# y9c/cutseq

Hardware: AMD Instinct MI355X
Metric: M read-pairs/sec (higher is better)
Workload: dtype u8

## Files before the change

### cutseq_amd/capi.py

```python
from __future__ import annotations

import ctypes as C
from pathlib import Path

from . import abi, switches

LIB_PATH = Path(__file__).with_name("libcutseq_hip.so")

EXPORTS = (
    "cs_abi_version", "cs_last_error", "cs_device_count", "cs_plan_create", "cs_plan_destroy", "cs_plan_set_demux", "cs_plan_set_demux_ops", "cs_plan_set_max_n",
    "cs_plan_set_max_length", "cs_plan_set_max_ee", "cs_plan_set_ee_reversed", "cs_xflag_counts_fetch", "cs_text_discards",
    "cs_engine_create", "cs_engine_destroy", "cs_trim_device", "cs_trim_device_pipelined", "cs_join", "cs_trim_batch", "cs_sync",
    "cs_stats_fetch", "cs_last_kernel_ms", "cs_last_kernel_split_ms", "cs_kernel_time_totals", "cs_alloc_pinned", "cs_alloc_pinned_huge", "cs_free_pinned", "cs_alloc_device",
    "cs_free_device", "cs_copy_to_device", "cs_copy_to_host",
    "cs_text_create", "cs_text_destroy", "cs_text_submit", "cs_text_wait", "cs_text_routes", "cs_text_fetch",
    "cs_text_info", "cs_text_fetch_info",
)


class HipUnavailable(RuntimeError):
    """The HIP extension (or a usable MI355X) is missing; the product has no CPU path."""


class CsError(RuntimeError):
    def __init__(self, code: int, message: str):
        super().__init__(f"cutseq_hip error {code}: {message}")
        self.code = code


_lib = None


def load() -> C.CDLL:
    global _lib
    if _lib is not None:
        return _lib
    lib_path = Path(switches.path("HIP_LIB", str(LIB_PATH)))
    if not lib_path.exists():
        raise HipUnavailable(
            f"{lib_path} not found: build it with `python -m cutseq_amd.build` "
            "(hipcc --offload-arch=gfx950). cutseq_amd has no CPU trimming path."
        )
    try:
        L = C.CDLL(str(lib_path))
    except OSError as exc:
        raise HipUnavailable(f"cannot load {lib_path}: {exc}") from exc
    vp, u32, i32 = C.c_void_p, C.c_uint32, C.c_int
    L.cs_abi_version.restype = i32
    L.cs_last_error.restype = C.c_char_p
    L.cs_device_count.restype = i32
    L.cs_plan_create.restype = i32
    L.cs_plan_create.argtypes = [vp, i32, vp, i32, C.POINTER(abi.cs_params), C.POINTER(vp)]
    L.cs_plan_set_demux.restype = i32
    L.cs_plan_set_demux.argtypes = [vp, i32, i32, vp, C.c_size_t]
    L.cs_plan_set_demux_ops.restype = i32
    L.cs_plan_set_demux_ops.argtypes = [vp, i32, i32, vp, i32]
    L.cs_plan_set_max_n.restype = i32
    L.cs_plan_set_max_n.argtypes = [vp, C.c_double]
    L.cs_plan_set_max_length.restype = i32
    L.cs_plan_set_max_length.argtypes = [vp, C.c_uint32]
    L.cs_plan_set_max_ee.restype = i32
    L.cs_plan_set_max_ee.argtypes = [vp, C.c_double]
    L.cs_plan_set_ee_reversed.restype = i32
    L.cs_plan_set_ee_reversed.argtypes = [vp, i32]
    L.cs_xflag_counts_fetch.restype = i32
    L.cs_xflag_counts_fetch.argtypes = [vp, vp, i32]
    L.cs_text_discards.restype = i32
    L.cs_text_discards.argtypes = [vp, C.c_uint32, vp]
    L.cs_plan_destroy.restype = None
    L.cs_plan_destroy.argtypes = [vp]
    L.cs_engine_create.restype = i32
    L.cs_engine_create.argtypes = [vp, i32, u32, u32, u32, C.POINTER(vp)]
    L.cs_engine_destroy.restype = None
    L.cs_engine_destroy.argtypes = [vp]
    L.cs_trim_device.restype = i32
    L.cs_trim_device.argtypes = [vp, vp, C.POINTER(abi.cs_reads), C.POINTER(abi.cs_reads), u32, u32]
    L.cs_trim_device_pipelined.restype = i32
    L.cs_trim_device_pipelined.argtypes = [vp, vp, C.POINTER(abi.cs_reads), C.POINTER(abi.cs_reads), u32, u32]
    L.cs_join.restype = i32
    L.cs_join.argtypes = [vp, vp]
    L.cs_trim_batch.restype = i32
    L.cs_trim_batch.argtypes = [vp, u32, C.POINTER(abi.cs_reads), C.POINTER(abi.cs_reads), u32, u32]
    L.cs_sync.restype = i32
    L.cs_sync.argtypes = [vp, u32]
    L.cs_stats_fetch.restype = i32
    L.cs_stats_fetch.argtypes = [vp, C.POINTER(abi.cs_stats * 2), i32]
    L.cs_last_kernel_ms.restype = i32
    L.cs_last_kernel_ms.argtypes = [vp, C.POINTER(C.c_float)]
    L.cs_last_kernel_split_ms.restype = i32
    L.cs_last_kernel_split_ms.argtypes = [vp, C.POINTER(C.c_float * 2)]
    L.cs_kernel_time_totals.restype = i32
    L.cs_kernel_time_totals.argtypes = [vp, C.POINTER(u32), C.POINTER(C.c_float * 2), i32]
    L.cs_alloc_pinned.restype = vp
    L.cs_alloc_pinned.argtypes = [C.c_size_t]
    L.cs_alloc_pinned_huge.restype = vp
    L.cs_alloc_pinned_huge.argtypes = [C.c_size_t]
    L.cs_free_pinned.restype = None
    L.cs_free_pinned.argtypes = [vp]
    L.cs_alloc_device.restype = vp
    L.cs_alloc_device.argtypes = [i32, C.c_size_t]
    L.cs_free_device.restype = None
    L.cs_free_device.argtypes = [i32, vp]
    L.cs_copy_to_device.restype = i32
    L.cs_copy_to_device.argtypes = [i32, vp, vp, C.c_size_t]
    L.cs_copy_to_host.restype = i32
    L.cs_copy_to_host.argtypes = [i32, vp, vp, C.c_size_t]
    u64 = C.c_uint64
    L.cs_text_create.restype = i32
    L.cs_text_create.argtypes = [vp, C.POINTER(abi.cs_text_params), u32, u64, u32, u32, C.POINTER(vp)]
    L.cs_text_destroy.restype = None
    L.cs_text_destroy.argtypes = [vp]
    L.cs_text_submit.restype = i32
    L.cs_text_submit.argtypes = [vp, u32, vp, u64, vp, u64, u32]
    L.cs_text_wait.restype = i32
    L.cs_text_wait.argtypes = [vp, u32, C.POINTER(abi.cs_text_result)]
    L.cs_text_routes.restype = i32
    L.cs_text_routes.argtypes = [vp, u32, vp, vp, vp]
# ... 27 lines not shown
```

### cutseq_amd/csrc/cutseq_hip.hip

```cpp
#include <hip/hip_runtime.h>

#include <cmath>
#include <cstdarg>
#include <cstdio>
#include <cstdlib>
#include <cstring>
#include <algorithm>
#include <atomic>
#include <map>
#include <new>
#include <string>
#include <thread>
#include <vector>

#include <sys/mman.h>

#include "../../include/cutseq_hip.h"
#include "trim_kernel.hip.inc"
#include "long_kernel.hip.inc"
#include "text_kernels.hip.inc"
#include "deflate_kernels.hip.inc"
#include "info_kernels.hip.inc"

namespace {
// ... 491 lines not shown
          d.fnib[idx >> 3] |= (uint32_t)((d.op.seq[d.op.reversed ? mm - 1 - idx : idx] >> 3) & 7u) << (4 * (idx & 7));
    }
  for (int m = 0; m < 2; ++m)
    for (int i = 0; i < cnt[m]; ++i) {
      csdev::DevOp &d = p->host.ops[m][i];
      if (d.op.kind != CS_OP_CUT) continue;
      auto pack = [](const cs_op &o) {
        return (uint32_t)(uint16_t)o.cut_len | ((uint32_t)(o.conditional ? 1u : 0u) << 16) | ((uint32_t)(o.capture & 3u) << 17) |
               ((uint32_t)(o.force_min_len > 0x1fff ? 0x1fffu : o.force_min_len) << 19);
      };
      d.cut_run = 1;
      d.cut_pack[0] = pack(d.op);
    }
  {
    const char *env = getenv("CUTSEQ_CUT_RUNS");
    if (!(env && atoi(env) == 0))
      for (int m = 0; m < 2; ++m)
        for (int i = 0; i < cnt[m];) {
          if (p->host.ops[m][i].op.kind != CS_OP_CUT) {
            ++i;
            continue;
          }
          int j = i;
          while (j < cnt[m] && j - i < csdev::kCutRun && p->host.ops[m][j].op.kind == CS_OP_CUT) {
            p->host.ops[m][i].cut_pack[j - i] = p->host.ops[m][j].cut_pack[0];
            ++j;
          }
          p->host.ops[m][i].cut_run = (uint32_t)(j - i);
          i = j;
        }
  }
  {
    const char *env = getenv("CUTSEQ_PAIR");
    const bool allow = coded && !(env && atoi(env) == 0);
    const char *env_log = getenv("CUTSEQ_LOG_ALWAYS");
    const bool log_always = env_log && atoi(env_log) != 0;
    auto log_friendly = [log_always](int mm, int kk) {
      if (log_always) return true;
      double variants = 0, choose = 1, pw = 1;
      for (int e = 0; e <= kk && e <= mm; ++e) {
        variants += choose * pw;
        choose = choose * (double)(mm - e) / (double)(e + 1);
        pw *= 6.0;
      }
      double space = 1;
      for (int i = 0; i < mm; ++i) space *= 4.0;
      return 300.0 * variants / space < 0.03;
    };
    for (int m = 0; m < 2; ++m) {
      if (allow && cnt[m] >= 1) {
        csdev::DevOp &f = p->host.ops[m][0];
        const bool free_ends = (f.op.align_flags & (CS_QUERY_START | CS_QUERY_STOP)) == (CS_QUERY_START | CS_QUERY_STOP);
        if (f.op.kind == CS_OP_ADAPTER && f.filter_mode == csdev::FILTER_MYERS32 && !f.op.reversed && free_ends &&
            f.op.shortcut == CS_SHORTCUT_NONE && !f.exists_only && log_friendly(f.op.m, f.op.k))
          f.solo_first = 1;
      }
      if (!allow || cnt[m] < 2) continue;
      csdev::DevOp &a = p->host.ops[m][0];
      const csdev::DevOp &b = p->host.ops[m][1];
      const int ma = a.op.m, ka = a.op.k, mo = a.op.min_overlap;
      const bool ends_free = (b.op.align_flags & (CS_QUERY_START | CS_QUERY_STOP)) == (CS_QUERY_START | CS_QUERY_STOP);
      if (!a.exists_only || a.op.kind != CS_OP_ADAPTER || b.op.kind != CS_OP_ADAPTER || b.exists_only ||
          b.filter_mode != csdev::FILTER_MYERS32 || b.op.reversed || !ends_free || b.op.shortcut != CS_SHORTCUT_NONE ||
          ma + ka > 31 || ka > 14 || !log_friendly(b.op.m, b.op.k))
        continue;
      a.pair_next = 1;
      for (int ent = 0; ent < 4; ++ent) {
        const int which = (ent == 0) ? 0 : (ent == 1) ? 1 : (ent == 2) ? 3 : 2;
        uint32_t fwd = 0;
        for (int i = 0; i < ma; ++i)
          if ((a.peq[which] >> (ma - 1 - i)) & 1ull) fwd |= 1u << i;
        a.eq_fwd[ent] = fwd << (32 - ma);
      }
      for (int j = 1; j <= 32; ++j) {
        int best = -1;
        if (j > ma + ka) best = ka;
        else
          for (int i = mo; i <= ma; ++i) {
            const int d = i > j ? i - j : j - i;
            if (d <= (int)a.op.thr[i] && (int)a.op.thr[i] > best) best = a.op.thr[i];
          }
        a.pair_tn[(j - 1) >> 3] |= (uint32_t)(best + 1) << (4 * ((j - 1) & 7));
      }
    }
  }
  *out = p;
  return CS_OK;
}

void cs_plan_destroy(cs_plan *plan) { delete plan; }

int cs_plan_set_max_n(cs_plan *plan, double count) {
  if (!plan) return fail(CS_ERR_ARG, "null plan");
  if (!(count >= 0.0)) return fail(CS_ERR_ARG, "max_n %g: the count must not be negative or NaN", count);
  plan->host.max_n_on = 1;
  plan->host.max_n = count;
  return CS_OK;
}

int cs_plan_set_max_length(cs_plan *plan, uint32_t length) {
  if (!plan) return fail(CS_ERR_ARG, "null plan");
  plan->host.max_length_on = 1;
  plan->host.max_length = length;
  return CS_OK;
}

int cs_plan_set_max_ee(cs_plan *plan, double errors) {
  if (!plan) return fail(CS_ERR_ARG, "null plan");
  if (!(errors >= 0.0)) return fail(CS_ERR_ARG, "max_ee %g: the bound must not be negative or NaN", errors);
  plan->host.max_ee_on = 1;
  plan->host.max_ee = errors;
  for (int b = 0; b < 256; ++b) plan->host.ee_table[b] = pow(10.0, (double)(33 - b) / 10.0);
  return CS_OK;
}

int cs_plan_set_ee_reversed(cs_plan *plan, int reversed) {
  if (!plan) return fail(CS_ERR_ARG, "null plan");
  plan->host.ee_reversed = reversed ? 1u : 0u;
  return CS_OK;
}

int cs_plan_set_demux(cs_plan *plan, int mate, int op_index, const uint16_t *table, size_t entries) {
  if (!plan || !table) return fail(CS_ERR_ARG, "null plan or table");
  if (mate < 1 || mate > 2 || op_index < 0 || op_index >= plan->host.n_ops[mate - 1])
    return fail(CS_ERR_ARG, "mate %d op %d: no such op", mate, op_index);
  const cs_op &op = plan->host.ops[mate - 1][op_index].op;
  if (op.kind != CS_OP_DEMUX) return fail(CS_ERR_ARG, "mate %d op %d is not a CS_OP_DEMUX op", mate, op_index);
  if (plan->host.ops[mate - 1][op_index].filter_mode)
    return fail(CS_ERR_ARG, "mate %d op %d: m + k = %d > %d (or CS_DEMUX_BY_OPS) takes cs_plan_set_demux_ops, not a table", mate,
                op_index, op.m + op.k, CS_DEMUX_MAX_PREFIX);
  size_t want = 0, pw = 1;
  for (int l = 0; l <= op.m + op.k; ++l, pw *= 5) want += pw;
  if (entries != want) return fail(CS_ERR_ARG, "demux table: %zu entries, expected %zu for m + k = %d", entries, want, op.m + op.k);
  try {
    plan->demux[mate - 1][op_index].assign(table, table + entries);
  } catch (const std::bad_alloc &) {
    return fail(CS_ERR_NOMEM, "out of memory");
  }
  return CS_OK;
}

namespace {

struct DemuxSegment {
  std::vector<uint8_t> pool;
  std::vector<std::pair<size_t, uint32_t>> first;
};

struct DemuxWalk {
  const std::vector<std::string> &digits;
  int m, k, depth;
  const std::vector<size_t> &block;

  struct Alive {
    int id;
    bool done;
    uint8_t col[CS_MAX_ADAPTER + 1];
  };
  struct Task {
    int len;
    size_t idx, pw, segment;
    std::vector<Alive> alive;
  };
  std::vector<std::vector<Alive>> scratch;
  DemuxSegment *seg = nullptr;
  bool overflow = false;
  int split = -1;
  std::vector<DemuxSegment> *segments = nullptr;
  std::vector<Task> *tasks = nullptr;

  void emit(size_t at, const std::vector<Alive> &alive) {
// ... 1299 lines not shown
```

### cutseq_amd/csrc/trim_kernel.hip.inc

```

#include <type_traits>

namespace csdev {

#ifdef CS_PHASE_TIMERS
struct PhaseTimer {
  uint64_t last;
  uint32_t acc[8];
  uint32_t passes, steps, items;
};
#define CS_T_MARK(T, PHASE)                                   \
  {                                                           \
    const uint64_t cs_now = clock64();                        \
    (T).acc[PHASE] += (uint32_t)(cs_now - (T).last);          \
    (T).last = cs_now;                                        \
  }
#else
#define CS_T_MARK(T, PHASE)
#endif


constexpr int kWave = 64;

constexpr uint32_t kScoreBias = 1024u, kOriginBias = 4096u;
constexpr uint32_t kCostShift = 24, kScoreShift = 13;
constexpr uint32_t kCellZero = (kScoreBias << kScoreShift) | kOriginBias;
constexpr uint32_t kDeltaMatch = 1u << kScoreShift;
constexpr uint32_t kDeltaMismatch = (1u << kCostShift) - (1u << kScoreShift);
constexpr uint32_t kDeltaIndel = (1u << kCostShift) - (2u << kScoreShift);

enum { FILTER_NONE = 0, FILTER_MYERS32 = 1, FILTER_MYERS64 = 2, FILTER_POLY_TAIL = 3, FILTER_POLY_HEAD = 4 };

__host__ __device__ constexpr uint32_t base_code(uint32_t ascii) {
  const uint32_t sel = (ascii >> 1) & 3u;
  const bool ok = ascii == 'A' || ascii == 'C' || ascii == 'G' || ascii == 'T';
  return (sel << 3) | (ok ? 0u : 32u);
}
constexpr int kEqTableBytes = 64;
constexpr int kWaveItemDwords = 4;
constexpr int kCutRun = 4;
constexpr int kQCutoffLow = -1, kQCutoffHigh = 256, kQTermMax = 256;

struct DevFields {
  uint32_t kind, align_flags, reversed, remove, shortcut, match_flag, required, conditional, capture, homopolymer,
      q_base, stat_slot, m, k, min_overlap, force_min_len;
  int32_t cut_len, q_cutoff;
};

struct DevOp {
  cs_op op;
  DevFields f;
  uint64_t peq[4];
  uint32_t filter_mode;
  uint32_t base_char;
  uint32_t acgt_only;
  uint32_t thr_mul;
  uint64_t thr_step[2];
  uint32_t eq_tab[kEqTableBytes / 4];
  uint32_t fnib[6];
  uint32_t exists_only;
  uint32_t pair_next;
  uint32_t solo_first;
  uint32_t pair_tn[4];
  uint32_t eq_fwd[4];
  uint32_t cut_run;
  uint32_t cut_pack[kCutRun];
};

struct DevPlan {
  cs_params params;
  int32_t n_ops[2];
  int32_t coded;
  int32_t max_n_on;
  DevOp ops[2][CS_MAX_OPS];
  double max_n;
  uint32_t max_length_on, max_length;
  uint32_t max_ee_on, ee_reversed;
  double max_ee;
  double ee_table[256];
};

constexpr int kMaxPlanSlots = 8;
__constant__ DevPlan c_plans[kMaxPlanSlots];

struct MateArgs {
  const uint32_t *seq;
  const uint8_t *qual;
  const uint16_t *len;
  cs_result *out;
  cs_cap2 *cap2;
  uint8_t *bc;
  uint8_t *xflags;
};

constexpr uint32_t kTileCounters = 8, kTileCounterStride = 32;

struct KArgs {
  MateArgs mate[2];
  unsigned long long *stats;
  uint32_t n_reads;
  uint32_t stride_dw;
  uint32_t lds_stride_dw;
  uint32_t col_dwords;
  uint32_t plan_slot;
  uint32_t *tile_counter;
  uint32_t n_table_ops;
  uint32_t big_tiles;
  uint32_t big_shift, small_shift;
  uint32_t static_units;
  uint4 *defer[2];
  uint32_t batch_knob;
  uint32_t *defer_count;
  uint32_t defer_cap;
  const unsigned long long *gate;
  uint32_t item_slots;
  uint32_t fast_recode;
};

__device__ __forceinline__ uint32_t cell_pack(int cost, int score, int origin) {
  return ((uint32_t)cost << kCostShift) | ((uint32_t)(score + (int)kScoreBias) << kScoreShift) |
// ... 881 lines not shown
  const uint32_t fill_a = (uint32_t)sha, cst4 = (uint32_t)(4 + 2 * ka + 1);
  auto sample_a = [&](uint32_t cst) {
    const int cur = (int)__builtin_popcount(sa.Pv) - (int)(__builtin_popcount(sa.Mv) + fill_a);
    flag |= sa.score + cur - (int)cst;
    sa.score = cur;
  };
  const unsigned long long tn_lo = ((unsigned long long)tn1 << 32) | tn0, tn_hi = ((unsigned long long)tn3 << 32) | tn2;
  auto tn_of = [tn_lo, tn_hi, ka](int j) -> int {
    int t1 = ka + 1;
    if (__ballot(j <= 32)) {
      const unsigned long long w = j <= 16 ? tn_lo : tn_hi;
      const int tj = (int)((uint32_t)(w >> (((uint32_t)(j - 1) & 15u) * 4u)) & 15u);
      t1 = j > 32 ? t1 : tj;
    }
    return t1;
  };
  auto column = [&](uint32_t eb, uint32_t ea, int j) {
    myers_step_la<false>(st, eb, 0u);
    if constexpr (HAS_A) {
      myers_step_la<false>(sa, ea, 0u);
      flag |= sa.score - tn_of(j);
    }
    if (st.score < 0) {
      if (jfirst < 0) jfirst = j;
      jlast = j;
      if (j == jmin + 1 && st.score + k1 == cmin) tie_next = true;
      if (st.score + k1 < cmin) {
        cmin = st.score + k1;
        jmin = j;
        tie_next = false;
      }
    }
  };
  int j = 1;
  if (n >= NB) {
    int wi = 0;
    auto take = [&]() -> uint32_t { return row[wi]; };
    auto advance = [&]() { wi += 1; };
#ifndef CS_PAIR_DEPTH
#define CS_PAIR_DEPTH 2
#endif
    constexpr int QD = CS_PAIR_DEPTH;
    static_assert(NB % QD == 0, "a group's columns must map onto the slots the same way in every group");
    uint32_t qb[QD], qa[QD];
    auto refill = [&](int slot, uint32_t code) {
      const unsigned long long pr = lds_read_u64(code);
      qb[slot] = (uint32_t)pr;
      qa[slot] = (uint32_t)(pr >> 32);
    };
    uint32_t wcur = take();
    advance();
#pragma unroll
    for (int u = 0; u < QD; ++u) refill(u, word_code<true>(wcur, u));
    auto group = [&](auto early_tag, uint32_t tw) {
      constexpr bool EARLY = decltype(early_tag)::value;
      const uint32_t wnext = take();
      advance();
      int sc[NB];
#pragma unroll
      for (int u = 0; u < NB; ++u) {
        myers_step_la<false>(st, qb[u % QD], 0u);
        sc[u] = st.score;
        if constexpr (HAS_A && EARLY) {
          myers_step_la<false>(sa, qa[u % QD], 0u);
          flag |= sa.score - (int)((tw >> (4 * u)) & 15u);
        } else if constexpr (HAS_A) {
          myers_step_noscore<false>(sa, qa[u % QD], 0u);
          if (u == 3 || u == 7) sample_a(cst4);
        }
        refill(u % QD, u + QD < NB ? word_code<true>(wcur, u + QD) : word_code<true>(wnext, u + QD - NB));
      }
      wcur = wnext;
      constexpr uint32_t kOr3 = 0xFEu;
      uint32_t any = __builtin_amdgcn_bitop3_b32((uint32_t)sc[0], (uint32_t)sc[1], (uint32_t)sc[2], kOr3);
      any = __builtin_amdgcn_bitop3_b32(any, (uint32_t)sc[3], (uint32_t)sc[4], kOr3);
      any = __builtin_amdgcn_bitop3_b32(any, (uint32_t)sc[5], (uint32_t)sc[6], kOr3);
      any |= (uint32_t)sc[7];
      if ((int)any < 0) {
        if (slot < slot_end) {
#pragma unroll
          for (int u = 0; u < NB; ++u) lds_write_u8(slot, (uint32_t)u, (uint32_t)sc[u]);
          lds_write_u8((slot >> 3) + il.tag_off, 0u, (uint32_t)(j >> 3));
        }
        slot += 8u;
      }
      j += NB;
    };
    __builtin_amdgcn_s_setprio(PRIO_LOOP);
    const int early_groups = (ma + ka + NB - 1) >> 3;
    if constexpr (HAS_A) {
      int g = 0;
      do {
        group(std::true_type{}, g == 0 ? tn0 : g == 1 ? tn1 : g == 2 ? tn2 : tn3);
        ++g;
      } while (g < early_groups && j + NB - 1 <= n);
    }
    while (j + NB - 1 <= n) group(std::false_type{}, 0u);
    __builtin_amdgcn_s_setprio(PRIO_REST);
    if (j <= n) {
      int sc[NB];
#pragma unroll
      for (int u = 0; u < NB - 1; ++u) {
        sc[u] = 0x7f;
        if (j + u <= n) {
          uint32_t eb, ea;
          if (u < QD) {
            eb = qb[u];
            ea = qa[u];
          } else {
            const unsigned long long pr = lds_read_u64(word_code<true>(wcur, u));
            eb = (uint32_t)pr;
            ea = (uint32_t)(pr >> 32);
          }
          myers_step_la<false>(st, eb, 0u);
          sc[u] = st.score;
          if constexpr (HAS_A) {
            myers_step_la<false>(sa, ea, 0u);
            flag |= sa.score - tn_of(j + u);
          }
        }
      }
      sc[NB - 1] = 0x7f;
      int any = sc[0];
#pragma unroll
      for (int u = 1; u < NB - 1; ++u) any |= sc[u];
      if (any < 0) {
        if (slot < slot_end) {
#pragma unroll
          for (int u = 0; u < NB; ++u) lds_write_u8(slot, (uint32_t)u, (uint32_t)sc[u]);
          lds_write_u8((slot >> 3) + il.tag_off, 0u, (uint32_t)(j >> 3));
        }
        slot += 8u;
      }
      j = n + 1;
    }
    {
      const uint32_t m80 = 0x80808080u, ones = 0x01010101u;
      const uint32_t stop_at = min(slot, slot_end);
      uint32_t rd = il.slot0;
      while (__ballot(rd < stop_at)) {
        if (rd < stop_at) {
          const unsigned long long sc8 = lds_read_u64(rd);
          const int jg = (int)lds_read_u8((rd >> 3) + il.tag_off) * 8 + 1;
          rd += 8u;
          const uint32_t clo = (uint32_t)sc8 & m80, chi = (uint32_t)(sc8 >> 32) & m80;
          const uint32_t plo = (uint32_t)sc8 ^ m80, phi = (uint32_t)(sc8 >> 32) ^ m80;
          const unsigned long long c64 = ((unsigned long long)chi << 32) | clo;
          if (jfirst < 0) jfirst = jg + (__builtin_ctzll(c64) >> 3);
          jlast = jg + ((63 - __builtin_clzll(c64)) >> 3);
          const uint32_t h00ff = 0x00ff00ffu;
// ... 708 lines not shown
        }
      }
    }
  }

  CS_T_MARK(pt, 7);
  const bool scan = do_end && j1 == n && max_n == n;
  if (works && scan) {
#pragma unroll
    for (int h = 0; h < H; ++h)
      if (rb + h + 1 <= top) fin[slot * fin_stride + rb + h + 1] = L[h];
  }
  wave_lds_fence();
  if (works && g == owner) {
    if (scan && !broke) {
      const int first_i = RE ? 1 : m;
      uint32_t todo = i3 & (top >= 32 ? 0xffffffffu : ((1u << top) - 1u)) & ~((1u << (first_i - 1)) - 1u);
      while (todo) {
        const int i = 32 - __builtin_clz(todo);
        todo &= ~(1u << (i - 1));
        const uint32_t c = fin[slot * fin_stride + i];
        if (c >= live_limit) continue;
        const int cost = cell_cost(c), score = strip_score(c), origin = cell_origin(c);
        const int length = i + min(origin, 0);
        if (length < min_overlap || length < 0) continue;
        if (cost > thr_of(d, length)) continue;
        const int b_length = b_refstop + min(b_origin, 0);
        if (better_candidate(rule, m, have, b_origin, b_cost, b_score, b_length, cost, score, origin, length)) {
          have = true;
          b_origin = origin;
          b_cost = cost;
          b_score = score;
          b_refstop = i;
          b_qstop = n;
        }
      }
    }
    const uint32_t qs = (uint32_t)(b_origin >= 0 ? b_origin : 0);
    wq[idx * kWaveItemDwords + 3] = ((have ? 1u : 0u) << 31) | (qs << 16) | (uint32_t)b_qstop;
  }
  wave_lds_fence();
}

__device__ __forceinline__ uint32_t wave_sum(uint32_t v) {
  int x = (int)v;
  x += __builtin_amdgcn_update_dpp(0, x, 0x111 , 0xf, 0xf, true);
  x += __builtin_amdgcn_update_dpp(0, x, 0x112 , 0xf, 0xf, true);
  x += __builtin_amdgcn_update_dpp(0, x, 0x114 , 0xf, 0xf, true);
  x += __builtin_amdgcn_update_dpp(0, x, 0x118 , 0xf, 0xf, true);
  x += __builtin_amdgcn_update_dpp(0, x, 0x142 , 0xa, 0xf, true);
  x += __builtin_amdgcn_update_dpp(0, x, 0x143 , 0xc, 0xf, true);
  return (uint32_t)__builtin_amdgcn_readlane(x, 63);
}
__device__ __forceinline__ uint32_t wave_count(bool p) { return (uint32_t)__popcll(__ballot(p)); }

__device__ __forceinline__ uint32_t atomic_add_later(uint32_t *p, uint32_t v) {
  uint32_t zero = 0;
  asm volatile("" : "+v"(zero));
  return atomicAdd(p + zero, v);
}


enum { ST_READS = 0, ST_IN_BP, ST_OUT_BP, ST_QTRIM_BP, ST_TOO_SHORT, ST_UNTRIMMED, ST_EXACT_DP, ST_RESERVED, ST_OPS };
constexpr int ST_TOO_MANY_N = ST_OPS + CS_MAX_OPS;
constexpr int kStatWords = ST_TOO_MANY_N + 1;
static_assert(sizeof(cs_stats) == kStatWords * 8, "cs_stats layout");
enum { XST_TOO_LONG = 0, XST_TOO_MANY_EE, kXStatWords };
constexpr int kXStatBase = 2 * kStatWords;
constexpr int kStatsBlockWords = kXStatBase + 2 * kXStatWords;

__device__ __forceinline__ uint32_t count_n_bytes(const uint32_t *row, int s, int e) {
  uint32_t n = 0;
  if (e <= s) return 0;
  const int d0 = s >> 2, d1 = (e - 1) >> 2;
  for (int d = d0; d <= d1; ++d) {
    uint32_t keep = 0x80808080u;
    if (d == d0) keep &= 0x80808080u << ((s & 3) * 8);
    if (d == d1) keep &= 0x80808080u >> ((3 - ((e - 1) & 3)) * 8);
    const uint32_t x = (row[d] & 0xdfdfdfdfu) ^ 0x4e4e4e4eu;
    n += (uint32_t)__popc(~(((x & 0x7f7f7f7fu) + 0x7f7f7f7fu) | x) & keep);
  }
  return n;
}
__device__ __forceinline__ uint32_t count_n_nibbles(const uint32_t *row, int s, int e) {
  uint32_t n = 0;
  if (e <= s) return 0;
  const int d0 = s >> 3, d1 = (e - 1) >> 3;
  for (int d = d0; d <= d1; ++d) {
    uint32_t keep = 0x11111111u;
    if (d == d0) keep &= 0x11111111u << ((s & 7) * 4);
    if (d == d1) keep &= 0x11111111u >> ((7 - ((e - 1) & 7)) * 4);
    const uint32_t w = row[d];
    n += (uint32_t)__popc(w & (w >> 1) & (w >> 2) & keep);
  }
  return n;
}
__device__ __forceinline__ bool too_many_n(uint32_t n, int len, double count) {
  if (count < 1.0) return len > 0 && (double)n / (double)len > count;
  return (double)n > count;
}
__device__ __forceinline__ double expected_errors(const uint32_t *qrow, int s, int e, const double *table, bool reversed) {
  double ee = 0.0;
  if (e <= s) return ee;
  const int d0 = s >> 2, d1 = (e - 1) >> 2;
  if (!reversed) {
    for (int d = d0; d <= d1; ++d) {
      const uint32_t w = qrow[d];
#pragma unroll
      for (int b = 0; b < 4; ++b) {
        const int p = 4 * d + b;
        if (p >= s && p < e) ee += table[(w >> (8 * b)) & 0xffu];
      }
    }
  } else {
    for (int d = d1; d >= d0; --d) {
      const uint32_t w = qrow[d];
#pragma unroll
      for (int b = 3; b >= 0; --b) {
        const int p = 4 * d + b;
        if (p >= s && p < e) ee += table[(w >> (8 * b)) & 0xffu];
      }
    }
  }
  return ee;
}

enum { MODE_SCAN = 0, MODE_RESOLVE = 1 };

#ifndef CS_SCAN_WAVES
#define CS_SCAN_WAVES 5
#endif
enum { FILT_NONE = 0, FILT_MAXN = 1, FILT_ALL = 2, FILT_ENDS = 3, FILT_NEXTSEQ = 4 };
template <bool CODED, bool WIDE, int MODE, int FILT>
__global__ void __launch_bounds__(64, MODE == MODE_RESOLVE ? 4 : CS_SCAN_WAVES) trim_kernel(KArgs a) {
  if (a.gate && *a.gate != ~0ull) return;
  const DevPlan *plan = &c_plans[a.plan_slot];
  extern __shared__ uint32_t smem[];
  constexpr int TILE = kWave;
  constexpr bool SCAN = MODE != MODE_RESOLVE;
  const int tid = threadIdx.x;
  const int mate = blockIdx.y;
  const MateArgs &ma = a.mate[mate];
  const int n_ops = plan->n_ops[mate];
  const uint32_t pw0 = (uint32_t)__builtin_amdgcn_readfirstlane((int)reinterpret_cast<const uint32_t *>(&plan->params)[1]);
  const uint32_t pw1 = (uint32_t)__builtin_amdgcn_readfirstlane((int)reinterpret_cast<const uint32_t *>(&plan->params)[2]);
  static_assert(offsetof(cs_params, min_length) == 4 && offsetof(cs_params, select_rule) == 6 && offsetof(cs_params, use_filter) == 7 &&
                offsetof(cs_params, case_rule) == 8 && offsetof(cs_params, indel_tie) == 9, "cs_params layout");
  const int min_length = (int)(pw0 & 0xffffu);
  const int rule = (int)((pw0 >> 16) & 0xffu);
  const bool use_filter = ((pw0 >> 24) & 0xffu) != 0;
  const bool fold_case = (pw1 & 0xffu) == CS_CASE_FOLD;
  const bool tie_ins = ((pw1 >> 8) & 0xffu) == CS_TIE_INSERTION;
  const int lane = tid;

  if (lds_addr_of(smem) != 0u) __builtin_trap();
  __builtin_amdgcn_s_setprio(SCAN ? PRIO_REST : PRIO_RESOLVE);
  uint32_t *cur_tab = smem;
  uint32_t *tile = smem + 20;
  uint32_t *col = tile + (size_t)TILE * a.lds_stride_dw;
  uint32_t *wq = col + a.col_dwords;
  uint32_t *tables = wq + (SCAN ? 0 : kWave * kWaveItemDwords);
  uint32_t *fnibs = tables + a.n_table_ops * (kEqTableBytes / 4);
  uint32_t *sacc = fnibs + a.n_table_ops * kFnibDwords;
  (void)col;
  (void)wq;

  for (int i = tid; i < (int)a.n_table_ops * (kEqTableBytes / 4); i += TILE) {
    const int t = i >> 4;
    tables[i] = t < n_ops ? plan->ops[mate][t].eq_tab[i & 15] : 0u;
  }
  for (int i = tid; i < (int)a.n_table_ops * kFnibDwords; i += TILE) {
    const int t = i / kFnibDwords, w = i - t * kFnibDwords;
    fnibs[i] = (CODED && t < n_ops) ? plan->ops[mate][t].fnib[w] : 0u;
  }
  for (int i = tid; i < kStatWords; i += TILE) sacc[i] = 0;
  if (SCAN && CODED && tid < 4) smem[16 + tid] = (n_ops > 0 && plan->ops[mate][0].pair_next) ? plan->ops[mate][0].eq_fwd[tid] : 0u;

  const uint32_t n_records = SCAN ? 0u : a.defer_count[mate * kTileCounterStride];
  uint32_t batch_rows = TILE;
  if (!SCAN) {
    if (n_records < a.batch_knob * 64u * (uint32_t)gridDim.x) batch_rows = 32;
    if (n_records < a.batch_knob * 32u * (uint32_t)gridDim.x) batch_rows = 16;
  }
  const uint32_t n_refl = SCAN ? 0u : a.defer_count[(4u + (uint32_t)mate) * kTileCounterStride];
  const uint32_t tiles_a = (n_records + batch_rows - 1) / batch_rows;
  const uint32_t n_tiles = SCAN ? (a.n_reads + (uint32_t)TILE - 1) / (uint32_t)TILE : tiles_a + (n_refl + (uint32_t)TILE - 1) / (uint32_t)TILE;
  const uint32_t big_tiles = a.big_tiles, big_units = big_tiles >> a.big_shift;
  const uint32_t big_mask = (1u << a.big_shift) - 1u, small_mask = (1u << a.small_shift) - 1u;
  auto unit_start = [&](uint32_t u) -> uint32_t {
    return (u < big_units) ? (u << a.big_shift) : big_tiles + ((u - big_units) << a.small_shift);
  };
  auto unit_end = [&](uint32_t tile) -> uint32_t {
    return (tile < big_tiles) ? ((tile | big_mask) + 1u) : big_tiles + (((tile - big_tiles) | small_mask) + 1u);
  };
  uint32_t *next_slot = sacc + kStatWords;
  const uint32_t n_counters = min(kTileCounters, (uint32_t)gridDim.x);
  const uint32_t my_counter = blockIdx.x % n_counters;
  uint32_t *counter = a.tile_counter + ((uint32_t)mate * kTileCounters + my_counter) * kTileCounterStride;
  uint32_t *claim = a.defer_count + (2u + (uint32_t)mate) * kTileCounterStride;
  auto next_unit = [&]() -> uint32_t { return a.static_units + my_counter + n_counters * atomicAdd(counter, 1u); };
  if (SCAN) {
    if (tid == 0) *next_slot = unit_start(blockIdx.x < a.static_units ? blockIdx.x : next_unit());
  } else {
    if (tid == 0) *next_slot = atomicAdd(claim, 1u);
  }
  __syncthreads();
  uint32_t tile_id = *next_slot, next_id = 0;
#ifdef CS_PHASE_TIMERS
  PhaseTimer pt;
  pt.last = clock64();
  for (int i = 0; i < 8; ++i) pt.acc[i] = 0;
  pt.passes = pt.steps = pt.items = 0;
#endif

  uint4 *ring = reinterpret_cast<uint4 *>((reinterpret_cast<uintptr_t>(sacc + kStatWords + 4) + 15u) & ~(uintptr_t)15u);
  uint32_t pend_count = 0;
  bool pend_asked = false;
  uint32_t pend_q = 0;
  auto flush_ring = [&]() {
    const uint32_t qb = (uint32_t)__builtin_amdgcn_readfirstlane((int)pend_q);
    if ((uint32_t)lane < pend_count) {
      uint4 *rec = a.defer[mate] + (size_t)(qb + (uint32_t)lane) * 2u;
      rec[0] = ring[lane * 2];
      rec[1] = ring[lane * 2 + 1];
    }
    pend_count = 0;
    pend_asked = false;
  };
  bool fast_ok = SCAN && CODED && a.fast_recode != 0u, fast_failed = false;
  for (; tile_id < n_tiles; tile_id = next_id) {
  uint32_t lane_fresh = threadIdx.x;
  asm volatile("" : "+v"(lane_fresh));
  const int tid = (int)lane_fresh, lane = tid;
  const bool top = !SCAN && tile_id >= tiles_a;
  const uint32_t row0 = top ? (tile_id - tiles_a) * (uint32_t)TILE : tile_id * batch_rows;
  const uint32_t rows_here = top ? min((uint32_t)TILE, n_refl - row0) : min(batch_rows, (SCAN ? a.n_reads : n_records) - row0);
  const bool valid = (uint32_t)tid < rows_here;

  uint32_t gr = row0 + tid;
  int s = 0, e = 0, t0 = 0;
  uint32_t fm = 0, capo = 0, qc = 0;
  uint32_t meta = (uint32_t)CS_DEMUX_NONE << 16;
  uint32_t rec_win = 0, rec_rows = 0, rec_rmax = 0;
  if (!SCAN) {
    uint4 ra = make_uint4(0, 0, 0, 0), rb = make_uint4(0, 0, 0, 0);
    if (valid) {
      const uint4 *rec = a.defer[mate] + (size_t)(top ? a.defer_cap - 1u - gr : gr) * 2u;
      ra = rec[0];
      rb = rec[1];
    }
    gr = ra.x;
    s = (int)(ra.y & 0xffffu);
    e = (int)(ra.y >> 16);
    rec_win = ra.z;
    rec_rows = ra.w;
    t0 = (int)(rb.x >> 24);
    fm = (rb.y & 0xffu) | ((rb.x & 0xffffffu) << 8);
    meta = ((rb.y >> 8) & 0xffu) | ((rb.w >> 24) << 16);
    rec_rmax = (rb.y >> 16) & 0xffu;
    capo = rb.z;
    qc = ((rb.w >> 8) & 0xffffu) | ((rb.y >> 24) << 16) | (rb.w << 24);
  }

  const uint32_t len_raw = valid ? (uint32_t)ma.len[gr] : 0u;
  const bool here = SCAN ? (valid && len_raw != (uint32_t)CS_LEN_SKIP) : valid;
  const int len = here ? min((int)len_raw, (int)(a.stride_dw * 4u)) : 0;

  {
    const uint32_t S = a.stride_dw;
    const uint32_t tile_b = lds_addr_of(tile);
    if (SCAN) {
      const uint32_t total = rows_here * S;
      const uint32_t *src = ma.seq + (size_t)row0 * S;
      if (CODED) {
        const uint32_t pad2 = (a.lds_stride_dw * 2u - S) * 2u;
        auto stage_coded = [&](auto fast_tag) -> uint32_t {
        constexpr bool FAST = decltype(fast_tag)::value;
        uint32_t bad = 0, done = 0;
        EncodeConsts ec;
        FastEncodeConsts fc;
        if constexpr (FAST) fc = fast_encode_consts(); else ec = encode_consts(fold_case);
        auto enc8 = [&](uint32_t w0, uint32_t w1) -> uint32_t {
          if constexpr (FAST) return encode8_nib_fast(w0, w1, bad, fc); else return encode8_nib_v(w0, w1, ec);
        };
        auto enc4 = [&](uint32_t w) -> uint32_t {
          if constexpr (FAST) return encode4_nib_fast(w, bad, fc); else return encode4_nib_v(w, ec);
        };
        if ((((uintptr_t)src) & 15u) == 0 && S >= 4) {
          const uint32_t quads = total >> 2;
          const uint4 *src4 = reinterpret_cast<const uint4 *>(src);
          constexpr int kBatch = 4;
          uint32_t r = (uint32_t)(((float)((uint32_t)tid << 2) + 0.5f) * (1.0f / (float)S)), c = ((uint32_t)tid << 2) - r * S;
          const uint32_t step_r = ((uint32_t)TILE << 2) / S, step_c = ((uint32_t)TILE << 2) - step_r * S;
          uint32_t dst = tile_b + ((uint32_t)tid << 3) + r * pad2;
          const uint32_t step_dst = ((uint32_t)TILE << 3) + step_r * pad2;
          const uint32_t last_q = quads - 1u;
          constexpr uint32_t kRound = (uint32_t)TILE * kBatch;
          uint4 w[kBatch];
#pragma unroll
          for (int u = 0; u < kBatch; ++u) w[u] = src4[min((uint32_t)tid + (uint32_t)u * TILE, last_q)];
          auto put = [&](const uint4 &v) {
            if (pad2 == 0) {
              *(lds_u64 *)(uintptr_t)dst = (unsigned long long)enc8(v.x, v.y) | ((unsigned long long)enc8(v.z, v.w) << 32);
            } else {
              const uint32_t n0 = enc4(v.x), n1 = enc4(v.y);
              const uint32_t n2 = enc4(v.z), n3 = enc4(v.w);
              lds_write_u16(dst, 0, n0);
              lds_write_u16(dst + ((c + 1 >= S) ? pad2 : 0u), 2, n1);
              lds_write_u16(dst + ((c + 2 >= S) ? pad2 : 0u), 4, n2);
              lds_write_u16(dst + ((c + 3 >= S) ? pad2 : 0u), 6, n3);
            }
          };
          auto step = [&]() {
            c += step_c;
            dst += step_dst;
            if (c >= S) {
              c -= S;
              dst += pad2;
            }
          };
          uint32_t qb = 0;
          for (; qb + kRound < quads; qb += kRound) {
#pragma unroll
            for (int u = 0; u < kBatch; ++u) {
              put(w[u]);
              step();
              w[u] = src4[min(qb + kRound + (uint32_t)u * TILE + (uint32_t)tid, last_q)];
            }
          }
#pragma unroll
          for (int u = 0; u < kBatch; ++u) {
            if (qb + (uint32_t)u * TILE + (uint32_t)tid < quads) put(w[u]);
            step();
          }
          done = quads << 2;
        }
        for (uint32_t dw = done + tid; dw < total; dw += TILE) {
          const uint32_t r = dw / S;
          lds_write_u16(tile_b + dw * 2u + r * pad2, 0, enc4(src[dw]));
        }
        return bad;
        };
        bool redo = !fast_ok;
        if (fast_ok) {
          const uint32_t bad = stage_coded(std::true_type{});
          if (a.fast_recode != 2u && __ballot(bad != 0u)) {
            redo = true;
            fast_ok = !fast_failed;
          }
          fast_failed = redo;
        }
        if (redo) (void)stage_coded(std::false_type{});
      } else {
        for (uint32_t dw = tid; dw < total; dw += TILE) {
          const uint32_t r = dw / S;
          tile[r * a.lds_stride_dw + (dw - r * S)] = fold_case ? upper4(src[dw]) : src[dw];
        }
      }
    } else {
      wq[tid] = gr;
      wave_lds_fence();
      const uint32_t total = rows_here * S;
      EncodeConsts ec = encode_consts(fold_case);
      uint32_t r = (uint32_t)tid / S, c = (uint32_t)tid - r * S;
      const uint32_t step_r = (uint32_t)TILE / S, step_c = (uint32_t)TILE - step_r * S;
      constexpr int kBatch = 8;
      for (uint32_t i0 = tid; i0 < total; i0 += (uint32_t)TILE * kBatch) {
        uint32_t w[kBatch], dst[kBatch];
#pragma unroll
        for (int u = 0; u < kBatch; ++u) {
          const uint32_t i = i0 + (uint32_t)u * TILE;
          if (i < total) {
            w[u] = ma.seq[(size_t)wq[r] * S + c];
            dst[u] = CODED ? (tile_b + r * a.lds_stride_dw * 4u + c * 2u) : (r * a.lds_stride_dw + c);
          }
          r += step_r;
          c += step_c;
          if (c >= S) {
            c -= S;
            r += 1;
          }
        }
#pragma unroll
        for (int u = 0; u < kBatch; ++u) {
          const uint32_t i = i0 + (uint32_t)u * TILE;
          if (i < total) {
            if (CODED)
              lds_write_u16(dst[u], 0, encode4_nib_v(w[u], ec));
            else
              tile[dst[u]] = fold_case ? upper4(w[u]) : w[u];
          }
        }
      }
      wave_lds_fence();
    }
  }
  __syncthreads();
  CS_T_MARK(pt, 0);
  const bool same_unit = SCAN && tile_id + 1 < unit_end(tile_id);
  uint32_t fetched = 0;
  if (tid == 0 && !same_unit) fetched = SCAN ? atomic_add_later(counter, 1u) : atomic_add_later(claim, 1u);
  if (SCAN && pend_count >= (uint32_t)kRingRecords / 2) {
    if (tid == 0) pend_q = atomic_add_later(&a.defer_count[mate * kTileCounterStride], pend_count);
    pend_asked = true;
  }
// ... 787 lines not shown
      atomicAdd(&sacc[ST_UNTRIMMED], w_untr);
      atomicAdd(&sacc[ST_EXACT_DP], w_exact);
    }
    for (int t = 0; t < n_ops; ++t) {
      const unsigned long long bal = __ballot(fin && ((fm >> (8 + t)) & 1u));
      if (lane == 0 && bal) atomicAdd(&sacc[ST_OPS + plan->ops[mate][t].f.stat_slot], (uint32_t)__popcll(bal));
    }
  }

  if (SCAN && refl_any) {
    const uint32_t qb = (uint32_t)__builtin_amdgcn_readfirstlane((int)refl_q);
    if (refl) {
      uint4 ra, rb;
      ra.x = gr;
      ra.y = (uint32_t)s | ((uint32_t)e << 16);
      ra.z = rec_win;
      ra.w = rec_rows;
      rb.x = (fm >> 8) | (meta & 0xff000000u);
      rb.y = (fm & 0xffu) | ((meta & 0xffu) << 8) | ((rec_rmax & 0xffu) << 16) | ((qc << 8) & 0xff000000u);
      rb.z = capo;
      rb.w = (qc >> 24) | ((qc & 0xffffu) << 8) | ((meta << 8) & 0xff000000u);
      uint4 *rec = a.defer[mate] + (size_t)(a.defer_cap - 1u - (qb + refl_rank)) * 2u;
      rec[0] = ra;
      rec[1] = rb;
    }
  }
  if (SCAN && pend_asked) flush_ring();
  if (SCAN && def_mask) {
    if (!park) q_pos = (uint32_t)__builtin_amdgcn_readfirstlane((int)q_pos);
    if (deferred && !refl) {
      const uint32_t rank = __builtin_amdgcn_mbcnt_hi((uint32_t)(def_mask >> 32),
                                                      __builtin_amdgcn_mbcnt_lo((uint32_t)def_mask, 0u));
      uint4 ra, rb;
      ra.x = gr;
      ra.y = (uint32_t)s | ((uint32_t)e << 16);
      ra.z = rec_win;
      ra.w = rec_rows;
      rb.x = (fm >> 8) | (meta & 0xff000000u);
      rb.y = (fm & 0xffu) | ((meta & 0xffu) << 8) | ((rec_rmax & 0xffu) << 16) | ((qc << 8) & 0xff000000u);
      rb.z = capo;
      rb.w = (qc >> 24) | ((qc & 0xffffu) << 8) | ((meta << 8) & 0xff000000u);
      uint4 *rec = park ? ring + (pend_count + rank) * 2u : a.defer[mate] + (size_t)(q_pos + rank) * 2u;
      rec[0] = ra;
      rec[1] = rb;
    }
    if (park) pend_count += (uint32_t)__popcll(def_mask);
  }
  next_id = same_unit ? tile_id + 1 : SCAN ? unit_start(a.static_units + my_counter + n_counters * fetched) : fetched;
  next_id = (uint32_t)__builtin_amdgcn_readfirstlane((int)next_id);
  __syncthreads();
  CS_T_MARK(pt, 6);
  }
  if (SCAN && pend_count) {
    if (!pend_asked && tid == 0) pend_q = atomicAdd(&a.defer_count[mate * kTileCounterStride], pend_count);
    flush_ring();
  }
#ifdef CS_PHASE_TIMERS
  if ((CS_PHASE_TIMERS == 1) == SCAN) {
    if (lane == 0)
      for (int i = 0; i < 8; ++i) atomicAdd(&sacc[ST_OPS + 16 + i], pt.acc[i] >> 6);
    if (lane == 0) {
      atomicAdd(&sacc[ST_OPS + 13], pt.passes);
      atomicAdd(&sacc[ST_OPS + 14], pt.steps);
      atomicAdd(&sacc[ST_OPS + 15], pt.items);
    }
  }
  __syncthreads();
#endif

  if (tid < kStatWords && sacc[tid])
    atomicAdd(&a.stats[(size_t)mate * kStatWords + tid], (unsigned long long)sacc[tid]);
}

}
```

### include/cutseq_hip.h

```cpp
#ifndef CUTSEQ_HIP_H
#define CUTSEQ_HIP_H

#include <stddef.h>
#include <stdint.h>

#ifdef __cplusplus
extern "C" {
#endif

#define CS_ABI_VERSION 7
#define CS_MAX_ADAPTER 128
#define CS_MAX_OPS 24
#define CS_MAX_STRIDE 1536
#define CS_LEN_SKIP 0xFFFF
#define CS_MAX_READ (1u << 24)

typedef enum cs_status {
  CS_OK = 0,
  CS_ERR_ARG = -1,
  CS_ERR_HIP = -2,
  CS_ERR_NO_GPU = -3,
  CS_ERR_NOMEM = -4,
  CS_ERR_STATE = -5
} cs_status;
// ... 95 lines not shown

typedef struct cs_cap2 {
  uint16_t off;
  uint8_t len;
  uint8_t _pad;
} cs_cap2;

typedef struct cs_stats {
  uint64_t n_reads;
  uint64_t in_bp;
  uint64_t out_bp;
  uint64_t qualtrim_bp;
  uint64_t n_too_short;
  uint64_t n_untrimmed;
  uint64_t n_exact_dp;
  uint64_t n_refiltered;
  uint64_t op_matched[CS_MAX_OPS];
  uint64_t n_too_many_n;
} cs_stats;

typedef struct cs_reads {
  const uint8_t *seq;
  const uint8_t *qual;
  const uint16_t *len;
  cs_result *out;
  cs_cap2 *cap2;
  uint8_t *bc;
  uint8_t *xflags;
} cs_reads;

typedef struct cs_plan cs_plan;
typedef struct cs_engine cs_engine;

int cs_abi_version(void);
const char *cs_last_error(void);
int cs_device_count(void);

int cs_plan_create(const cs_op *ops_r1, int n1, const cs_op *ops_r2, int n2, const cs_params *params,
                   cs_plan **out);
void cs_plan_destroy(cs_plan *plan);

int cs_plan_set_demux(cs_plan *plan, int mate, int op_index, const uint16_t *table, size_t entries);

int cs_plan_set_demux_ops(cs_plan *plan, int mate, int op_index, const cs_op *ops, int n_ops);

int cs_plan_set_max_n(cs_plan *plan, double count);

int cs_plan_set_max_length(cs_plan *plan, uint32_t length);

int cs_plan_set_max_ee(cs_plan *plan, double errors);

int cs_plan_set_ee_reversed(cs_plan *plan, int reversed);

int cs_engine_create(const cs_plan *plan, int device, uint32_t n_slots, uint32_t max_reads,
                     uint32_t max_stride, cs_engine **out);
void cs_engine_destroy(cs_engine *eng);

int cs_trim_device(cs_engine *eng, void *stream, const cs_reads *r1, const cs_reads *r2,
                   uint32_t n_reads, uint32_t stride);

int cs_trim_device_pipelined(cs_engine *eng, void *stream, const cs_reads *r1, const cs_reads *r2,
                             uint32_t n_reads, uint32_t stride);
int cs_join(cs_engine *eng, void *stream);

int cs_trim_batch(cs_engine *eng, uint32_t slot, const cs_reads *r1, const cs_reads *r2,
                  uint32_t n_reads, uint32_t stride);
int cs_sync(cs_engine *eng, uint32_t slot);

int cs_stats_fetch(cs_engine *eng, cs_stats stats[2], int reset);

int cs_xflag_counts_fetch(cs_engine *eng, uint64_t counts[2][CS_X_COUNTS], int reset);

int cs_last_kernel_ms(cs_engine *eng, float *ms);
int cs_last_kernel_split_ms(cs_engine *eng, float ms[2]);
int cs_kernel_time_totals(cs_engine *eng, uint32_t *calls, float ms[2], int reset);

enum {
  CS_TEXT_OK = 0,
  CS_TEXT_ERR_MALFORMED = 1,
  CS_TEXT_ERR_TOO_LONG = 2,
  CS_TEXT_ERR_IDS_DIFFER = 3,
  CS_TEXT_ERR_LINE_COUNT = 4,
  CS_TEXT_ERR_INFO_MISMATCH = 5,
  CS_TEXT_ERR_INFO_OVERFLOW = 6
};

enum {
  CS_INFO_ON = 1,
  CS_INFO_GZIP = 2,
  CS_INFO_NO_QUAL = 4
};

typedef struct cs_text_params {
  uint8_t has_umi;
  uint8_t untrimmed_filter;
  uint8_t reverse_complement;
  uint8_t compress;
  uint32_t max_tag;
  const char *suffix1[2];
  const char *suffix2[2];
  uint32_t n_bins;
  uint8_t fasta_out;
  uint8_t fasta_routes;
  uint8_t info;
  uint8_t too_long_route;
} cs_text_params;
// ... 43 lines not shown
```

Baseline: 4204.

## Skip score tracking in quiet Myers columns and specialize linear coded staging

```diff
diff --git a/cutseq_amd/capi.py b/cutseq_amd/capi.py
--- a/cutseq_amd/capi.py
+++ b/cutseq_amd/capi.py
@@ -9,7 +9,7 @@
 
 EXPORTS = (
     "cs_abi_version", "cs_last_error", "cs_device_count", "cs_plan_create", "cs_plan_destroy", "cs_plan_set_demux", "cs_plan_set_demux_ops", "cs_plan_set_max_n",
-    "cs_plan_set_max_length", "cs_plan_set_max_ee", "cs_plan_set_ee_reversed", "cs_xflag_counts_fetch", "cs_text_discards",
+    "cs_plan_set_max_length", "cs_plan_set_max_ee", "cs_plan_set_ee_reversed", "cs_plan_walk_info", "cs_xflag_counts_fetch", "cs_text_discards",
     "cs_engine_create", "cs_engine_destroy", "cs_trim_device", "cs_trim_device_pipelined", "cs_join", "cs_trim_batch", "cs_sync",
     "cs_stats_fetch", "cs_last_kernel_ms", "cs_last_kernel_split_ms", "cs_kernel_time_totals", "cs_alloc_pinned", "cs_alloc_pinned_huge", "cs_free_pinned", "cs_alloc_device",
     "cs_free_device", "cs_copy_to_device", "cs_copy_to_host",
@@ -63,6 +63,9 @@
     L.cs_plan_set_max_ee.argtypes = [vp, C.c_double]
     L.cs_plan_set_ee_reversed.restype = i32
     L.cs_plan_set_ee_reversed.argtypes = [vp, i32]
+    if hasattr(L, "cs_plan_walk_info"):
+        L.cs_plan_walk_info.restype = i32
+        L.cs_plan_walk_info.argtypes = [vp, i32, C.POINTER(u32 * 6)]
     L.cs_xflag_counts_fetch.restype = i32
     L.cs_xflag_counts_fetch.argtypes = [vp, vp, i32]
     L.cs_text_discards.restype = i32
diff --git a/cutseq_amd/csrc/cutseq_hip.hip b/cutseq_amd/csrc/cutseq_hip.hip
--- a/cutseq_amd/csrc/cutseq_hip.hip
+++ b/cutseq_amd/csrc/cutseq_hip.hip
@@ -567,8 +567,10 @@
         csdev::DevOp &f = p->host.ops[m][0];
         const bool free_ends = (f.op.align_flags & (CS_QUERY_START | CS_QUERY_STOP)) == (CS_QUERY_START | CS_QUERY_STOP);
         if (f.op.kind == CS_OP_ADAPTER && f.filter_mode == csdev::FILTER_MYERS32 && !f.op.reversed && free_ends &&
-            f.op.shortcut == CS_SHORTCUT_NONE && !f.exists_only && log_friendly(f.op.m, f.op.k))
+            f.op.shortcut == CS_SHORTCUT_NONE && !f.exists_only && log_friendly(f.op.m, f.op.k)) {
           f.solo_first = 1;
+          f.quiet_groups = (uint32_t)csdev::quiet_columns((int)f.op.align_flags, f.op.m, f.op.k, nullptr) / 8u;
+        }
       }
       if (!allow || cnt[m] < 2) continue;
       csdev::DevOp &a = p->host.ops[m][0];
@@ -597,6 +599,7 @@
           }
         a.pair_tn[(j - 1) >> 3] |= (uint32_t)(best + 1) << (4 * ((j - 1) & 7));
       }
+      a.quiet_groups = (uint32_t)csdev::quiet_columns((int)b.op.align_flags, b.op.m, b.op.k, a.pair_tn) / 8u;
     }
   }
   *out = p;
@@ -632,6 +635,18 @@
 int cs_plan_set_ee_reversed(cs_plan *plan, int reversed) {
   if (!plan) return fail(CS_ERR_ARG, "null plan");
   plan->host.ee_reversed = reversed ? 1u : 0u;
+  return CS_OK;
+}
+
+int cs_plan_walk_info(const cs_plan *plan, int mate, uint32_t info[6]) {
+  if (!plan || !info) return fail(CS_ERR_ARG, "null plan or info");
+  if (mate < 1 || mate > 2) return fail(CS_ERR_ARG, "mate %d: 1 or 2", mate);
+  memset(info, 0, 6 * sizeof info[0]);
+  if (plan->host.n_ops[mate - 1] < 1) return CS_OK;
+  const csdev::DevOp &a = plan->host.ops[mate - 1][0];
+  info[0] = a.pair_next ? 2u : a.solo_first ? 1u : 0u;
+  info[1] = a.quiet_groups;
+  for (int i = 0; i < 4; ++i) info[2 + i] = a.pair_tn[i];
   return CS_OK;
 }
 
diff --git a/cutseq_amd/csrc/trim_kernel.hip.inc b/cutseq_amd/csrc/trim_kernel.hip.inc
--- a/cutseq_amd/csrc/trim_kernel.hip.inc
+++ b/cutseq_amd/csrc/trim_kernel.hip.inc
@@ -65,7 +65,21 @@
   uint32_t eq_fwd[4];
   uint32_t cut_run;
   uint32_t cut_pack[kCutRun];
+  uint32_t quiet_groups;
 };
+
+__host__ __device__ inline int quiet_columns(int flags, int m, int k, const uint32_t *tn) {
+  if (flags & CS_REF_START) return 0;
+  int q = 0;
+  while (q + 8 < m - k && q + 8 <= 32) {
+    bool clear = true;
+    for (int j = q > 0 ? q : 1; j < q + 8 && tn; ++j)
+      clear = clear && ((tn[(j - 1) >> 3] >> (4 * ((j - 1) & 7))) & 15u) == 0u;
+    if (!clear) break;
+    q += 8;
+  }
+  return q;
+}
 
 struct DevPlan {
   cs_params params;
@@ -1053,10 +1067,22 @@
     advance();
 #pragma unroll
     for (int u = 0; u < QD; ++u) refill(u, word_code<true>(wcur, u));
-    auto group = [&](auto early_tag, uint32_t tw) {
-      constexpr bool EARLY = decltype(early_tag)::value;
+    constexpr int STEADY = 0, EARLY_G = 1, QUIET = 2;
+    auto group = [&](auto body_tag, uint32_t tw) {
+      constexpr bool EARLY = decltype(body_tag)::value == EARLY_G;
       const uint32_t wnext = take();
       advance();
+      if constexpr (decltype(body_tag)::value == QUIET) {
+#pragma unroll
+        for (int u = 0; u < NB; ++u) {
+          myers_step_noscore<false>(st, qb[u % QD], 0u);
+          if constexpr (HAS_A) myers_step_noscore<false>(sa, qa[u % QD], 0u);
+          refill(u % QD, u + QD < NB ? word_code<true>(wcur, u + QD) : word_code<true>(wnext, u + QD - NB));
+        }
+        wcur = wnext;
+        j += NB;
+        return;
+      }
       int sc[NB];
 #pragma unroll
       for (int u = 0; u < NB; ++u) {
@@ -1089,14 +1115,25 @@
     };
     __builtin_amdgcn_s_setprio(PRIO_LOOP);
     const int early_groups = (ma + ka + NB - 1) >> 3;
+    const int quiet_j = (int)da.quiet_groups * NB + 1;
+    if (quiet_j > 1) {
+      do group(std::integral_constant<int, QUIET>{}, 0u);
+      while (j < quiet_j && j + NB - 1 <= n);
+      st.score = (int)__builtin_popcount(st.Pv) - (int)(__builtin_popcount(st.Mv) + (uint32_t)sh) - k1;
+      if constexpr (HAS_A) {
+        sa.score = (int)__builtin_popcount(sa.Pv) - (int)(__builtin_popcount(sa.Mv) + fill_a);
+        const int tq = (int)(da.pair_tn[da.quiet_groups - 1u] >> 28);
+        flag |= sa.score - (j == quiet_j ? tq : 0);
+      }
+    }
     if constexpr (HAS_A) {
-      int g = 0;
-      do {
-        group(std::true_type{}, g == 0 ? tn0 : g == 1 ? tn1 : g == 2 ? tn2 : tn3);
+      int g = (int)da.quiet_groups;
+      while (g < early_groups && j + NB - 1 <= n) {
+        group(std::integral_constant<int, EARLY_G>{}, g == 0 ? tn0 : g == 1 ? tn1 : g == 2 ? tn2 : tn3);
         ++g;
-      } while (g < early_groups && j + NB - 1 <= n);
-    }
-    while (j + NB - 1 <= n) group(std::false_type{}, 0u);
+      }
+    }
+    while (j + NB - 1 <= n) group(std::integral_constant<int, STEADY>{}, 0u);
     __builtin_amdgcn_s_setprio(PRIO_REST);
     if (j <= n) {
       int sc[NB];
@@ -1911,6 +1948,11 @@
   x += __builtin_amdgcn_update_dpp(0, x, 0x143 , 0xc, 0xf, true);
   return (uint32_t)__builtin_amdgcn_readlane(x, 63);
 }
+__device__ __forceinline__ uint32_t wave_lane_fresh() {
+  uint32_t zero = 0u;
+  asm volatile("" : "+v"(zero));
+  return __builtin_amdgcn_mbcnt_hi(~0u, __builtin_amdgcn_mbcnt_lo(~0u, zero));
+}
 __device__ __forceinline__ uint32_t wave_count(bool p) { return (uint32_t)__popcll(__ballot(p)); }
 
 __device__ __forceinline__ uint32_t atomic_add_later(uint32_t *p, uint32_t v) {
@@ -2010,7 +2052,9 @@
   const bool use_filter = ((pw0 >> 24) & 0xffu) != 0;
   const bool fold_case = (pw1 & 0xffu) == CS_CASE_FOLD;
   const bool tie_ins = ((pw1 >> 8) & 0xffu) == CS_TIE_INSERTION;
+#ifdef CS_PHASE_TIMERS
   const int lane = tid;
+#endif
 
   if (lds_addr_of(smem) != 0u) __builtin_trap();
   __builtin_amdgcn_s_setprio(SCAN ? PRIO_REST : PRIO_RESOLVE);
@@ -2078,8 +2122,9 @@
   uint32_t pend_q = 0;
   auto flush_ring = [&]() {
     const uint32_t qb = (uint32_t)__builtin_amdgcn_readfirstlane((int)pend_q);
-    if ((uint32_t)lane < pend_count) {
-      uint4 *rec = a.defer[mate] + (size_t)(qb + (uint32_t)lane) * 2u;
+    const uint32_t lane = wave_lane_fresh();
+    if (lane < pend_count) {
+      uint4 *rec = a.defer[mate] + (size_t)(qb + lane) * 2u;
       rec[0] = ring[lane * 2];
       rec[1] = ring[lane * 2 + 1];
     }
@@ -2088,7 +2133,7 @@
   };
   bool fast_ok = SCAN && CODED && a.fast_recode != 0u, fast_failed = false;
   for (; tile_id < n_tiles; tile_id = next_id) {
-  uint32_t lane_fresh = threadIdx.x;
+  uint32_t lane_fresh = SCAN ? wave_lane_fresh() : threadIdx.x;
   asm volatile("" : "+v"(lane_fresh));
   const int tid = (int)lane_fresh, lane = tid;
   const bool top = !SCAN && tile_id >= tiles_a;
@@ -2133,8 +2178,9 @@
       const uint32_t *src = ma.seq + (size_t)row0 * S;
       if (CODED) {
         const uint32_t pad2 = (a.lds_stride_dw * 2u - S) * 2u;
-        auto stage_coded = [&](auto fast_tag) -> uint32_t {
-        constexpr bool FAST = decltype(fast_tag)::value;
+        const bool linear = pad2 == 0 && (((uintptr_t)src) & 15u) == 0 && S >= 4;
+        auto stage_coded = [&](auto fast_tag, auto linear_tag) -> uint32_t {
+        constexpr bool FAST = decltype(fast_tag)::value, LINEAR = decltype(linear_tag)::value;
         uint32_t bad = 0, done = 0;
         EncodeConsts ec;
         FastEncodeConsts fc;
@@ -2145,30 +2191,50 @@
         auto enc4 = [&](uint32_t w) -> uint32_t {
           if constexpr (FAST) return encode4_nib_fast(w, bad, fc); else return encode4_nib_v(w, ec);
         };
-        if ((((uintptr_t)src) & 15u) == 0 && S >= 4) {
+        constexpr int kBatch = 4;
+        constexpr uint32_t kRound = (uint32_t)TILE * kBatch;
+        if constexpr (LINEAR) {
+          const uint32_t quads = total >> 2, last_q = quads - 1u;
+          const uint4 *src4 = reinterpret_cast<const uint4 *>(src);
+          uint32_t dst = tile_b + ((uint32_t)tid << 3);
+          uint4 w[kBatch];
+#pragma unroll
+          for (int u = 0; u < kBatch; ++u) w[u] = src4[min((uint32_t)tid + (uint32_t)u * TILE, last_q)];
+          auto put = [&](const uint4 &v, uint32_t off) {
+            *(lds_u64 *)(uintptr_t)(dst + off) = (unsigned long long)enc8(v.x, v.y) | ((unsigned long long)enc8(v.z, v.w) << 32);
+          };
+          uint32_t qb = 0;
+          for (; qb + kRound < quads; qb += kRound) {
+#pragma unroll
+            for (int u = 0; u < kBatch; ++u) {
+              put(w[u], (uint32_t)u * TILE * 8u);
+              w[u] = src4[min(qb + kRound + (uint32_t)u * TILE + (uint32_t)tid, last_q)];
+            }
+            dst += kRound * 8u;
+          }
+#pragma unroll
+          for (int u = 0; u < kBatch; ++u)
+            if (qb + (uint32_t)u * TILE + (uint32_t)tid < quads) put(w[u], (uint32_t)u * TILE * 8u);
+          done = quads << 2;
+        } else if ((((uintptr_t)src) & 15u) == 0 && S >= 4) {
           const uint32_t quads = total >> 2;
           const uint4 *src4 = reinterpret_cast<const uint4 *>(src);
-          constexpr int kBatch = 4;
           uint32_t r = (uint32_t)(((float)((uint32_t)tid << 2) + 0.5f) * (1.0f / (float)S)), c = ((uint32_t)tid << 2) - r * S;
           const uint32_t step_r = ((uint32_t)TILE << 2) / S, step_c = ((uint32_t)TILE << 2) - step_r * S;
           uint32_t dst = tile_b + ((uint32_t)tid << 3) + r * pad2;
           const uint32_t step_dst = ((uint32_t)TILE << 3) + step_r * pad2;
           const uint32_t last_q = quads - 1u;
-          constexpr uint32_t kRound = (uint32_t)TILE * kBatch;
+          (void)enc8;
           uint4 w[kBatch];
 #pragma unroll
           for (int u = 0; u < kBatch; ++u) w[u] = src4[min((uint32_t)tid + (uint32_t)u * TILE, last_q)];
           auto put = [&](const uint4 &v) {
-            if (pad2 == 0) {
-              *(lds_u64 *)(uintptr_t)dst = (unsigned long long)enc8(v.x, v.y) | ((unsigned long long)enc8(v.z, v.w) << 32);
-            } else {
-              const uint32_t n0 = enc4(v.x), n1 = enc4(v.y);
-              const uint32_t n2 = enc4(v.z), n3 = enc4(v.w);
-              lds_write_u16(dst, 0, n0);
-              lds_write_u16(dst + ((c + 1 >= S) ? pad2 : 0u), 2, n1);
-              lds_write_u16(dst + ((c + 2 >= S) ? pad2 : 0u), 4, n2);
-              lds_write_u16(dst + ((c + 3 >= S) ? pad2 : 0u), 6, n3);
-            }
+            const uint32_t n0 = enc4(v.x), n1 = enc4(v.y);
+            const uint32_t n2 = enc4(v.z), n3 = enc4(v.w);
+            lds_write_u16(dst, 0, n0);
+            lds_write_u16(dst + ((c + 1 >= S) ? pad2 : 0u), 2, n1);
+            lds_write_u16(dst + ((c + 2 >= S) ? pad2 : 0u), 4, n2);
+            lds_write_u16(dst + ((c + 3 >= S) ? pad2 : 0u), 6, n3);
           };
           auto step = [&]() {
             c += step_c;
@@ -2200,16 +2266,19 @@
         }
         return bad;
         };
+        auto stage = [&](auto fast_tag) -> uint32_t {
+          return linear ? stage_coded(fast_tag, std::true_type{}) : stage_coded(fast_tag, std::false_type{});
+        };
         bool redo = !fast_ok;
         if (fast_ok) {
-          const uint32_t bad = stage_coded(std::true_type{});
+          const uint32_t bad = stage(std::true_type{});
           if (a.fast_recode != 2u && __ballot(bad != 0u)) {
             redo = true;
             fast_ok = !fast_failed;
           }
           fast_failed = redo;
         }
-        if (redo) (void)stage_coded(std::false_type{});
+        if (redo) (void)stage(std::false_type{});
       } else {
         for (uint32_t dw = tid; dw < total; dw += TILE) {
           const uint32_t r = dw / S;
@@ -3103,7 +3172,7 @@
   CS_T_MARK(pt, 6);
   }
   if (SCAN && pend_count) {
-    if (!pend_asked && tid == 0) pend_q = atomicAdd(&a.defer_count[mate * kTileCounterStride], pend_count);
+    if (!pend_asked && wave_lane_fresh() == 0u) pend_q = atomicAdd(&a.defer_count[mate * kTileCounterStride], pend_count);
     flush_ring();
   }
 #ifdef CS_PHASE_TIMERS
@@ -3119,8 +3188,9 @@
   __syncthreads();
 #endif
 
-  if (tid < kStatWords && sacc[tid])
-    atomicAdd(&a.stats[(size_t)mate * kStatWords + tid], (unsigned long long)sacc[tid]);
-}
-
-}
+  const int tid_end = SCAN ? (int)wave_lane_fresh() : tid;
+  if (tid_end < kStatWords && sacc[tid_end])
+    atomicAdd(&a.stats[(size_t)mate * kStatWords + tid_end], (unsigned long long)sacc[tid_end]);
+}
+
+}
diff --git a/include/cutseq_hip.h b/include/cutseq_hip.h
--- a/include/cutseq_hip.h
+++ b/include/cutseq_hip.h
@@ -171,6 +171,8 @@
 
 int cs_plan_set_ee_reversed(cs_plan *plan, int reversed);
 
+int cs_plan_walk_info(const cs_plan *plan, int mate, uint32_t info[6]);
+
 int cs_engine_create(const cs_plan *plan, int device, uint32_t n_slots, uint32_t max_reads,
                      uint32_t max_stride, cs_engine **out);
 void cs_engine_destroy(cs_engine *eng);
```

Result: faster. 4264, median of 6 (+1.4%).
